# hideki1217/rusTfhe

Hardware: AMD Instinct MI355X
Metric: HomNAND gates/sec (whole node), N=1024 (higher is better)
Workload: dtype f64

## Files before the change

### rustfhe_amd/csrc/rtfhe_body_pair_rr.hpp

```cpp
    typedef PairRrLds S;
    constexpr int LOGN = 10, SLOTS = S::SLOTS;
    typedef Geo<LOGN> G;
    constexpr int N = G::N, P = G::P, R = G::R, NT = 128 * SLOTS;
    constexpr uint32_t MA = decomp_add(L, BGBIT, decltype(tvs)::ROUNDED), MX = decomp_xor(L, BGBIT, decltype(tvs)::ROUNDED);
    static_assert(L == 3, "three rows per side are held in registers");
    extern __shared__ __align__(16) unsigned char smem[];
    const int tid = threadIdx.x, lane = tid & 63;
    const int wave = __builtin_amdgcn_readfirstlane(tid >> 6);
    const int slot = wave % SLOTS;
    const int side = wave / SLOTS;
    const int per = a.count / (int)gridDim.x, extra = a.count % (int)gridDim.x, wg = (int)blockIdx.x;
    const int gc = per + (wg < extra ? 1 : 0);
    const int g_first = wg * per + (wg < extra ? wg : extra);
    if (gc < SLOTS || gc > S::GMAX) return;

    cplx* tw = reinterpret_cast<cplx*>(smem);
    for (int idx = tid; idx < G::TW_TOTAL; idx += NT) tw[idx] = a.tw[idx];
    const cplx* twf = tw;
    const cplx* twi = tw + G::TW_DIR;

    unsigned char* sbase = smem + S::TW + (size_t)slot * S::SLOT;
    double* xb0 = reinterpret_cast<double*>(sbase);
    double* xb1 = xb0 + 2 * G::XSLOTS;
    double* myx = side ? xb1 : xb0;
    cplx* hand0 = reinterpret_cast<cplx*>(xb0) + lane;
    cplx* hand1 = reinterpret_cast<cplx*>(xb1) + lane;
    uint32_t* flags = reinterpret_cast<uint32_t*>(sbase + 2 * S::XB);
    uint32_t* done = reinterpret_cast<uint32_t*>(smem + S::TW + SLOTS * S::SLOT);
    unsigned char* gates0 = smem + S::TW + SLOTS * S::SLOT + S::DONE;
    const size_t gate_bytes = S::gate_bytes(a.npad);
    if (lane == 0) flags[side] = 0u;
    if (tid < 2 * S::GMAX) done[tid] = 0u;
    const unsigned my_flag = (unsigned)__builtin_amdgcn_readfirstlane((int)(unsigned)(size_t)(__attribute__((address_space(3))) uint32_t*)(flags + side));
    const unsigned partner_flag = (unsigned)__builtin_amdgcn_readfirstlane((int)(unsigned)(size_t)(__attribute__((address_space(3))) uint32_t*)(flags + (1 - side)));
    const unsigned done_side = (unsigned)__builtin_amdgcn_readfirstlane((int)(unsigned)(size_t)(__attribute__((address_space(3))) uint32_t*)(done + side));

    const int n = a.n;
    for (int gl = 0; gl < gc; gl++) {
        constexpr int SH = 32 - LOGN - 1;
        const GateIo io = gate_io(a, g_first + gl);
        uint16_t* ab = reinterpret_cast<uint16_t*>(gates0 + gl * gate_bytes + (size_t)2 * N * 4);
        for (int i = tid; i <= n; i += NT) {
            const uint32_t t = gate_linear(io.op, io.p0[i], io.p1[i], i == n);
            if constexpr (decltype(tvs)::MANY) ab[i] = (uint16_t)mod_switch<SH>(t, i == n, tv_shift(tvs));
            else ab[i] = (uint16_t)((i == n) ? (t >> SH) : ((t + (1u << (SH - 1))) >> SH));
        }
    }
    __syncthreads();
    for (int gl = 0; gl < gc; gl++) {
        uint32_t* acc = reinterpret_cast<uint32_t*>(gates0 + gl * gate_bytes);
        const auto tv = tv_row(tvs, g_first + gl, N);
        const int bbar = (int)reinterpret_cast<const uint16_t*>(acc + 2 * N)[n];
        for (int c = tid; c < N; c += NT) {
            const int e = (c + bbar) & (2 * N - 1);
            acc[c] = tv_word<LOGN>(tv, e);
            if constexpr (decltype(tvs)::ENC) acc[N + c] = tv_word_a<LOGN>(tv, e);
            else acc[N + c] = 0u;
        }
    }
    __syncthreads();

    const size_t trgsw_cplx = (size_t)2 * L * 2 * R * 64;
    cplx bA[R], bB[R];
    typedef unsigned int v4u __attribute__((ext_vector_type(4)));
    const __amdgpu_buffer_rsrc_t bk_rsrc = __builtin_amdgcn_make_buffer_rsrc(const_cast<cplx*>(a.bk), 0, 0x7fffffff, 0x00020000);
    const int lane16 = lane * 16;
    auto fetch = [&](cplx (&dst)[R], int step, int rc) {
        const size_t row = (size_t)step * trgsw_cplx + (size_t)((side * L + rc % L) * 2 + rc / L) * R * 64;
        const int s_lo = __builtin_amdgcn_readfirstlane((int)(row * sizeof(cplx)));
        const int s_hi = s_lo + (R / 2) * 64 * (int)sizeof(cplx);
        __builtin_amdgcn_sched_barrier(0);
#pragma unroll
        for (int m = 0; m < R / 2; m++) {
            const v4u v = __builtin_amdgcn_raw_buffer_load_b128(bk_rsrc, lane16 + m * 1024, s_lo, 0);
            dst[m] = make_double2(__longlong_as_double(((unsigned long long)v.y << 32) | v.x), __longlong_as_double(((unsigned long long)v.w << 32) | v.z));
        }
#pragma unroll
        for (int m = 0; m < R / 2; m++) {
            const v4u v = __builtin_amdgcn_raw_buffer_load_b128(bk_rsrc, lane16 + m * 1024, s_hi, 0);
            dst[R / 2 + m] = make_double2(__longlong_as_double(((unsigned long long)v.y << 32) | v.x), __longlong_as_double(((unsigned long long)v.w << 32) | v.z));
        }
        __builtin_amdgcn_sched_barrier(0);
    };
    if (a.steps > 0) {
        fetch(bA, 0, side ? 0 : 1);
        fetch(bB, 0, side ? 1 : 0);
    }
    constexpr int LOWER_AT = 2, RAISE_AT = 10;
    auto prio_point = [&](int point) {
        if (point == LOWER_AT) asm volatile("s_cmp_lg_u32 %0, 0\n\ts_cbranch_scc1 1f\n\ts_setprio 0\n1:" ::"s"(side) : "scc");
        if (point == RAISE_AT) asm volatile("s_cmp_lg_u32 %0, 0\n\ts_cbranch_scc1 1f\n\ts_setprio 2\n1:" ::"s"(side) : "scc");
    };
    if (side) __builtin_amdgcn_s_setprio(1); else __builtin_amdgcn_s_setprio(2);
    unsigned seq = 0;
    int gl = slot, i = 0;
#pragma unroll 1
    while (i < a.steps) {
        int gl2 = gl + SLOTS, i2 = i;
        if (gl2 >= gc) { gl2 -= gc; i2++; }
        const int nxt = (i2 < a.steps) ? i2 : i;
        uint32_t* poly = reinterpret_cast<uint32_t*>(gates0 + gl * gate_bytes) + side * N;
        const int r = __builtin_amdgcn_readfirstlane((int)reinterpret_cast<const uint16_t*>(gates0 + gl * gate_bytes + (size_t)2 * N * 4)[i]);
        const unsigned done_flag = done_side + 8u * (unsigned)gl;
        flag_wait(done_flag, (unsigned)i);
        int ln = lane;
        asm volatile("" : "+v"(ln));
        uint32_t own[2 * R], u[2 * R];
#pragma unroll
        for (int mm = 0; mm < 2 * R; mm++) own[mm] = poly[ln + 64 * mm];
        rotated_gather(u, own, poly, ln, r, MA, MX);
        double xr[L][R], xi[L][R];
#pragma unroll
        for (int jj = 0; jj < L; jj++) {
#pragma unroll
            for (int m = 0; m < R; m++) {
                xr[jj][m] = (double)decomp_digit(u[m], BGBIT, jj);
                xi[jj][m] = (double)decomp_digit(u[R + m], BGBIT, jj);
            }
        }
        auto pp1 = [&]() { prio_point(1); };
        fft_forward_multi_a<LOGN, L, true, decltype(pp1), true>(xr, xi, twf, myx, myx + G::XSLOTS, ln, pp1);
        prio_point(2);
        fft_forward_multi_b<LOGN, L, BOOT_TRIV>(xr, xi, twf);
        prio_point(5);

        double sre[R], sim[R];
        auto zero = [&]() {
#pragma unroll
            for (int m = 0; m < R; m++) { sre[m] = 0.0; sim[m] = 0.0; }
        };
        auto put = [&](cplx* h) {
#pragma unroll
            for (int m = 0; m < R; m++) h[m * 64] = make_double2(sre[m], sim[m]);
        };
        auto get = [&](const cplx* h) {
#pragma unroll
            for (int m = 0; m < R; m++) { const cplx v = h[m * 64]; sre[m] = v.x; sim[m] = v.y; }
        };

        if (side == 0) {
            mac_row_first<R>(sre, sim, bB, xr[0], xi[0]); fetch(bB, i, 2);
            mac_row<R>(sre, sim, bA, xr[1], xi[1]); fetch(bA, i, 3);
            mac_row<R>(sre, sim, bB, xr[2], xi[2]); fetch(bB, i, 4);
            put(hand0);
        }
        prio_point(6);
        seq++; flag_arrive(my_flag, seq); flag_wait(partner_flag, seq);
        prio_point(7);
        if (side == 0) zero(); else get(hand0);
        mac_row<R>(sre, sim, bA, xr[0], xi[0]); fetch(bA, i, side ? 2 : 5);
        mac_row<R>(sre, sim, bB, xr[1], xi[1]); fetch(bB, side ? i : nxt, side ? 3 : 0);
        mac_row<R>(sre, sim, bA, xr[2], xi[2]); fetch(bA, side ? i : nxt, side ? 4 : 1);
        put(side ? hand0 : hand1);
        prio_point(8);
        seq++; flag_arrive(my_flag, seq); flag_wait(partner_flag, seq);
        prio_point(9);
        if (side == 1) {
            get(hand1);
            mac_row<R>(sre, sim, bB, xr[0], xi[0]); fetch(bB, i, 5);
            mac_row<R>(sre, sim, bA, xr[1], xi[1]); fetch(bA, nxt, 0);
            mac_row<R>(sre, sim, bB, xr[2], xi[2]); fetch(bB, nxt, 1);
        } else {
            get(hand0);
        }

        fft_inverse<LOGN, 1, BOOT_TRIV>(sre, sim, twi, twi, myx, lane);
#pragma unroll
        for (int m = 0; m < R; m++) {
            const int c = lane + 64 * m;
            poly[c] = own[m] + trunc_to_torus(sre[m]);
            poly[c + P] = own[R + m] + trunc_to_torus(sim[m]);
        }
        wave_lds_sync();
        flag_arrive(done_flag, (unsigned)i + 1u);
        prio_point(10);
        gl = gl2; i = i2;
    }
    __builtin_amdgcn_s_setprio(0);
    __syncthreads();

#define RR_PAIR_SYNC() do { seq++; flag_arrive(my_flag, seq); flag_wait(partner_flag, seq); } while (0)
#pragma unroll 1
    for (int ge_l = slot; ge_l < gc; ge_l += SLOTS) {
        const int g = g_first + ge_l;
        const GateIo io = gate_io(a, g, tvs);
        const bool live = io.ok;
        uint32_t* accbuf = reinterpret_cast<uint32_t*>(gates0 + ge_l * gate_bytes);
        uint32_t* poly = accbuf + side * N;
        if (a.mode == MODE_BLIND_ROTATE) {
            if (live) {
                uint32_t* o = a.out + (size_t)g * 2 * N + side * N;
                for (int c = lane; c < N; c += 64) o[c] = poly[c];
            }
            continue;
        }
        if (side == 1) {
            uint32_t av[2 * R];
#pragma unroll
            for (int mm = 0; mm < 2 * R; mm++) av[mm] = poly[lane + 64 * mm];
            wave_lds_sync();
#pragma unroll
            for (int mm = 0; mm < 2 * R; mm++) {
                const int c = lane + 64 * mm;
                poly[(N - c) & (N - 1)] = (c == 0) ? av[mm] : (0u - av[mm]);
            }
        }
        RR_PAIR_SYNC();
        if (a.mode == MODE_EXTRACT) {
            if constexpr (decltype(tvs)::MANY) {
                if (live) many_extract<N>(a.ext, a.ext_first + g, tv_shift(tvs), accbuf, side * (N / 2) + lane, (side + 1) * (N / 2), 64, side ? -1 : lane);
                continue;
            }
            if (live) {
                const int ge = a.ext_first + g;
                for (int c = side * (N / 2) + lane; c < (side + 1) * (N / 2); c += 64) *ext_slot(a.ext, ge, c, N) = accbuf[N + c];
                if (side == 0 && lane == 0) *ext_slot(a.ext, ge, N, N) = accbuf[0];
                for (int c = side * 64 + lane; c <= n; c += 128) io.out[c] = 0u;
            }
            continue;
        }
        uint4 sum[KSQ];
        ks_accumulate<LOGN, KS_T, KS_BB, KSQ>(accbuf + N, side * (N / 2), (side + 1) * (N / 2), a.ksk, a.ksw, sum, lane);
        uint4* part = reinterpret_cast<uint4*>(xb1) + lane;
        if (side == 1) {
#pragma unroll
            for (int q = 0; q < KSQ; q++) part[q * 64] = sum[q];
        }
        RR_PAIR_SYNC();
        if (side == 0 && live) {
            const uint32_t bprime = accbuf[0];
            uint32_t* out = io.out;
#pragma unroll
            for (int q = 0; q < KSQ; q++) {
                const uint4 o = part[q * 64];
                const int col = 4 * (lane + 64 * q);
                const uint32_t s[4] = {sum[q].x + o.x, sum[q].y + o.y, sum[q].z + o.z, sum[q].w + o.w};
#pragma unroll
                for (int e = 0; e < 4; e++)
                    if (col + e <= n) out[col + e] = ((col + e == n) ? bprime : 0u) - s[e];
            }
        }
        RR_PAIR_SYNC();
    }
#undef RR_PAIR_SYNC
```

### rustfhe_amd/csrc/rtfhe_device.hpp

```cpp
#pragma once

#include <hip/hip_runtime.h>
#include <stdint.h>

namespace rtfhe {

typedef double2 cplx;

constexpr bool BOOT_TRIV = true;

__host__ __device__ constexpr int ilog2(int v) { return v <= 1 ? 0 : 1 + ilog2(v >> 1); }

template <int LOGN>
struct Geo {
    static constexpr int N = 1 << LOGN;
    static constexpr int P = N / 2;
    static constexpr int LOGP = LOGN - 1;
    static constexpr int R = P / 64;
    static constexpr int LR = ilog2(R);
    static constexpr int LOW = LOGP - 2 * LR;
    static constexpr int NLOW = 1 << LOW;
    static_assert(LOW >= 2 && LOW <= LR, "supported: N = 1024, 2048");
    static constexpr int TW_TWIST = 0;
    static constexpr int TW_P1 = TW_TWIST + R * 64;
    static constexpr int TW_P2 = TW_P1 + (R - 1) * 64;
    static constexpr int TW_P3 = TW_P2 + (R - 1) * NLOW;
    static constexpr int TW_DIR = TW_P3 + (NLOW - 4);
    static constexpr int TW_TOTAL = 2 * TW_DIR;
    static constexpr int XSLOTS = P + 64;
    __host__ __device__ static constexpr int f1(int pos) { return pos + NLOW * (pos >> 6); }
    __host__ __device__ static constexpr int f2(int pos) { return pos + (pos >> LR); }
    __host__ __device__ static constexpr int pos1(int lane, int m) { return lane + 64 * m; }
    __host__ __device__ static constexpr int pos2(int lane, int m) {
        return ((lane >> LOW) << 6) | (m << LOW) | (lane & (NLOW - 1));
    }
    __host__ __device__ static constexpr int pos3(int lane, int m) { return (lane << LR) | m; }
};

__device__ __forceinline__ void wave_lds_sync() {
    __builtin_amdgcn_fence(__ATOMIC_RELEASE, "wavefront");
    __builtin_amdgcn_wave_barrier();
    __builtin_amdgcn_fence(__ATOMIC_ACQUIRE, "wavefront");
}

__device__ __forceinline__ void lds_st(double* p, double v) {
    __hip_atomic_store(p, v, __ATOMIC_RELAXED, __HIP_MEMORY_SCOPE_WAVEFRONT);
}
__device__ __forceinline__ double lds_ld(const double* p) {
    return __hip_atomic_load(p, __ATOMIC_RELAXED, __HIP_MEMORY_SCOPE_WAVEFRONT);
}
__device__ __forceinline__ void lds_st128(cplx* p, double re, double im) { *p = make_double2(re, im); }
__device__ __forceinline__ cplx lds_ld128(const cplx* p) { return *p; }


template <int CNT>
struct Tw {
    cplx w[CNT > 0 ? CNT : 1];
    __device__ __forceinline__ void load(const cplx* __restrict__ tw, int stride) {
#pragma unroll
        for (int e = 0; e < CNT; e++) w[e] = tw[e * stride];
    }
};

template <int R, int MB, bool TRIV0 = false>
__device__ __forceinline__ void fwd_stage_tw(double (&re)[R], double (&im)[R], const cplx* w) {
    constexpr int h = 1 << MB;
#pragma unroll
    for (int m = 0; m < R; m++) {
        if (m & h) continue;
        const int m1 = m | h, q = m & (h - 1);
        const double sr = re[m] + re[m1], si = im[m] + im[m1];
        const double dr = re[m] - re[m1], di = im[m] - im[m1];
        re[m] = sr; im[m] = si;
        if (TRIV0 && q == 0) { re[m1] = dr; im[m1] = di; continue; }
        double a = dr * w[q].x, b = di * w[q].y;
        re[m1] = a - b;
        a = dr * w[q].y; b = di * w[q].x;
        im[m1] = a + b;
    }
}

template <int R, int MB, bool CONJ = false, bool TRIV0 = false>
__device__ __forceinline__ void inv_stage_tw(double (&re)[R], double (&im)[R], const cplx* w) {
    constexpr int h = 1 << MB;
#pragma unroll
    for (int m = 0; m < R; m++) {
        if (m & h) continue;
        const int m1 = m | h, q = m & (h - 1);
        if (TRIV0 && q == 0) {
            const double ar = re[m], ai = im[m], tr = re[m1], ti = im[m1];
            re[m] = ar + tr; im[m] = ai + ti;
            re[m1] = ar - tr; im[m1] = ai - ti;
            continue;
        }
        const double t0 = re[m1] * w[q].x, t1 = re[m1] * w[q].y, t2 = im[m1] * w[q].x, t3 = im[m1] * w[q].y;
        const double tr = CONJ ? t0 + t3 : t0 - t3, ti = CONJ ? t2 - t1 : t1 + t2;
        const double ar = re[m], ai = im[m];
        re[m] = ar + tr; im[m] = ai + ti;
        re[m1] = ar - tr; im[m1] = ai - ti;
    }
}

template <int R>
__device__ __forceinline__ void stage_size2(double (&re)[R], double (&im)[R]) {
#pragma unroll
    for (int m = 0; m < R; m += 2) {
        const double r0 = re[m], r1 = re[m + 1], j0 = im[m], j1 = im[m + 1];
        re[m] = r0 + r1; re[m + 1] = r0 + (-r1);
        im[m] = j0 + j1; im[m + 1] = j0 + (-j1);
    }
}

template <int R>
__device__ __forceinline__ void fwd_stage_size4(double (&re)[R], double (&im)[R]) {
#pragma unroll
    for (int m = 0; m < R; m += 4) {
        const double r0 = re[m], r1 = re[m + 1], r2 = re[m + 2], r3 = re[m + 3];
        const double j0 = im[m], j1 = im[m + 1], j2 = im[m + 2], j3 = im[m + 3];
        re[m] = r0 + r2; re[m + 1] = r1 + r3; re[m + 2] = r0 + (-r2); re[m + 3] = (-j1) + j3;
        im[m] = j0 + j2; im[m + 1] = j1 + j3; im[m + 2] = j0 + (-j2); im[m + 3] = r1 + (-r3);
    }
}

template <int R>
__device__ __forceinline__ void inv_stage_size4(double (&re)[R], double (&im)[R]) {
#pragma unroll
    for (int m = 0; m < R; m += 4) {
        const double r0 = re[m], r1 = re[m + 1], r2 = re[m + 2], r3 = re[m + 3];
        const double j0 = im[m], j1 = im[m + 1], j2 = im[m + 2], j3 = im[m + 3];
        re[m] = r0 + r2; re[m + 1] = r1 + j3;    re[m + 2] = r0 + (-r2); re[m + 3] = r1 + (-j3);
        im[m] = j0 + j2; im[m + 1] = j1 + (-r3); im[m + 2] = j0 + (-j2); im[m + 3] = j1 + r3;
    }
}

template <int R>
__device__ __forceinline__ void twist_mul(double (&re)[R], double (&im)[R], const cplx* w) {
#pragma unroll
    for (int m = 0; m < R; m++) {
        const double rc = re[m] * w[m].x, ic = im[m] * w[m].x, rs = re[m] * w[m].y, is = im[m] * w[m].y;
        re[m] = rc - is;
        im[m] = ic + rs;
    }
}

template <int R, int MBTOP>
struct P12 {
    __device__ __forceinline__ static void fwd(double (&re)[R], double (&im)[R], const cplx* w) {
        if constexpr (MBTOP >= 0) {
            constexpr int h = 1 << MBTOP;
            fwd_stage_tw<R, MBTOP>(re, im, w + (R - 2 * h));
            P12<R, MBTOP - 1>::fwd(re, im, w);
        }
    }
    template <bool CONJ = false>
    __device__ __forceinline__ static void inv(double (&re)[R], double (&im)[R], const cplx* w) {
        if constexpr (MBTOP >= 0) {
            constexpr int h = 1 << MBTOP;
            P12<R, MBTOP - 1>::template inv<CONJ>(re, im, w);
            inv_stage_tw<R, MBTOP, CONJ>(re, im, w + (R - 2 * h));
        }
    }
};

template <int R, int NLOW, int MBTOP, bool TRIV = false>
struct P3 {
    __device__ __forceinline__ static void fwd(double (&re)[R], double (&im)[R], const cplx* w) {
        if constexpr (MBTOP >= 2) {
            constexpr int h = 1 << MBTOP;
            fwd_stage_tw<R, MBTOP, TRIV>(re, im, w + (NLOW - 2 * h));
            P3<R, NLOW, MBTOP - 1, TRIV>::fwd(re, im, w);
        } else {
            fwd_stage_size4<R>(re, im);
            stage_size2<R>(re, im);
        }
    }
    template <bool CONJ = false>
    __device__ __forceinline__ static void inv(double (&re)[R], double (&im)[R], const cplx* w) {
        if constexpr (MBTOP >= 2) {
            constexpr int h = 1 << MBTOP;
            P3<R, NLOW, MBTOP - 1, TRIV>::template inv<CONJ>(re, im, w);
            inv_stage_tw<R, MBTOP, CONJ, TRIV>(re, im, w + (NLOW - 2 * h));
        } else {
            stage_size2<R>(re, im);
            inv_stage_size4<R>(re, im);
        }
    }
};

template <int LOGN, int FROM, int TO, int DUAL = 0>
__device__ __forceinline__ void exchange(double (&re)[Geo<LOGN>::R], double (&im)[Geo<LOGN>::R],
                                         double* __restrict__ xbuf, int lane, double* __restrict__ ximbuf = nullptr) {
    typedef Geo<LOGN> G;
    constexpr int R = G::R;
    auto slot = [&](int layout, int m) {
        const int pos = layout == 1 ? G::pos1(lane, m) : layout == 2 ? G::pos2(lane, m) : G::pos3(lane, m);
        return (FROM + TO == 3) ? G::f1(pos) : G::f2(pos);
    };
    if constexpr (DUAL && G::LR == G::LOW) {
        double* xim = ximbuf ? ximbuf : xbuf + G::XSLOTS;
        constexpr bool X12 = (FROM + TO == 3);
        auto base = [&](int layout) {
            return layout == 1 ? lane : layout == 2 ? (G::NLOW + 64) * (lane >> G::LOW) + (lane & (G::NLOW - 1)) : (R + 1) * lane;
        };
        auto stride = [](int layout) constexpr { return layout == 1 ? 64 + G::NLOW : layout == 2 ? (X12 ? G::NLOW : G::NLOW + 1) : 1; };
        static_assert(G::f1(G::pos1(5, 3)) == 5 + (64 + G::NLOW) * 3 && G::f2(G::pos3(5, 3)) == (R + 1) * 5 + 3, "affine slot maps");
        const int bw = base(FROM), br = base(TO);
        constexpr int sw = stride(FROM), sr = stride(TO);
        if constexpr (DUAL == 2) {
            cplx* xc = reinterpret_cast<cplx*>(xbuf);
#pragma unroll
            for (int m = 0; m < R; m++) lds_st128(&xc[bw + sw * m], re[m], im[m]);
            wave_lds_sync();
#pragma unroll
            for (int m = 0; m < R / 2; m++) {
                const cplx a = lds_ld128(&xc[br + sr * m]), b = lds_ld128(&xc[br + sr * (m + R / 2)]);
                re[m] = a.x; im[m] = a.y; re[m + R / 2] = b.x; im[m + R / 2] = b.y;
            }
            wave_lds_sync();
            return;
        }
#pragma unroll
        for (int m = 0; m < R; m++) lds_st(&xbuf[bw + sw * m], re[m]);
#pragma unroll
        for (int m = 0; m < R; m++) lds_st(&xim[bw + sw * m], im[m]);
        wave_lds_sync();
#pragma unroll
        for (int m = 0; m < R / 2; m++) {
            re[m] = lds_ld(&xbuf[br + sr * m]); re[m + R / 2] = lds_ld(&xbuf[br + sr * (m + R / 2)]);
            im[m] = lds_ld(&xim[br + sr * m]);  im[m + R / 2] = lds_ld(&xim[br + sr * (m + R / 2)]);
        }
        wave_lds_sync();
    } else if constexpr (DUAL) {
        double* xim = ximbuf ? ximbuf : xbuf + G::XSLOTS;
#pragma unroll
        for (int m = 0; m < R; m++) lds_st(&xbuf[slot(FROM, m)], re[m]);
#pragma unroll
        for (int m = 0; m < R; m++) lds_st(&xim[slot(FROM, m)], im[m]);
        wave_lds_sync();
#pragma unroll
        for (int m = 0; m < R / 2; m++) {
            re[m] = lds_ld(&xbuf[slot(TO, m)]); re[m + R / 2] = lds_ld(&xbuf[slot(TO, m + R / 2)]);
            im[m] = lds_ld(&xim[slot(TO, m)]);  im[m + R / 2] = lds_ld(&xim[slot(TO, m + R / 2)]);
        }
        wave_lds_sync();
    } else {
#pragma unroll
        for (int m = 0; m < R; m++) lds_st(&xbuf[slot(FROM, m)], re[m]);
        wave_lds_sync();
#pragma unroll
        for (int m = 0; m < R; m++) re[m] = lds_ld(&xbuf[slot(TO, m)]);
        wave_lds_sync();
#pragma unroll
        for (int m = 0; m < R; m++) lds_st(&xbuf[slot(FROM, m)], im[m]);
        wave_lds_sync();
#pragma unroll
        for (int m = 0; m < R; m++) im[m] = lds_ld(&xbuf[slot(TO, m)]);
        wave_lds_sync();
    }
}

template <int LOGN, int DUAL = 0>
__device__ __forceinline__ void fft_forward_a(double (&re)[Geo<LOGN>::R], double (&im)[Geo<LOGN>::R],
                                              const cplx* __restrict__ tw, double* __restrict__ xbuf, int lane,
                                              double* __restrict__ xim = nullptr) {
    typedef Geo<LOGN> G;
    constexpr int R = G::R;
    Tw<R> wt; Tw<R - 1> w1, w2;
    wt.load(tw + G::TW_TWIST + lane, 64);
    w1.load(tw + G::TW_P1 + lane, 64);
    twist_mul<R>(re, im, wt.w);
    P12<R, G::LR - 1>::fwd(re, im, w1.w);
    w2.load(tw + G::TW_P2 + (lane & (G::NLOW - 1)), G::NLOW);
    exchange<LOGN, 1, 2, DUAL>(re, im, xbuf, lane, xim);
    P12<R, G::LR - 1>::fwd(re, im, w2.w);
}
template <int LOGN, int DUAL = 0, bool TRIV = false>
__device__ __forceinline__ void fft_forward_b(double (&re)[Geo<LOGN>::R], double (&im)[Geo<LOGN>::R],
                                              const cplx* __restrict__ tw, double* __restrict__ xbuf, int lane,
                                              double* __restrict__ xim = nullptr) {
    typedef Geo<LOGN> G;
    Tw<G::NLOW - 4> w3;
    w3.load(tw + G::TW_P3, 1);
    exchange<LOGN, 2, 3, DUAL>(re, im, xbuf, lane, xim);
    P3<G::R, G::NLOW, G::LOW - 1, TRIV>::fwd(re, im, w3.w);
}
template <int LOGN, int DUAL = 0, bool TRIV = false>
__device__ __forceinline__ void fft_forward(double (&re)[Geo<LOGN>::R], double (&im)[Geo<LOGN>::R],
                                            const cplx* __restrict__ tw, double* __restrict__ xbuf, int lane,
                                            double* __restrict__ xim = nullptr) {
    fft_forward_a<LOGN, DUAL>(re, im, tw, xbuf, lane, xim);
    fft_forward_b<LOGN, DUAL, TRIV>(re, im, tw, xbuf, lane, xim);
}

template <int LOGN, int FROM, int TO, bool B128 = false>
struct XAffine {
    typedef Geo<LOGN> G;
    static_assert(G::LR == G::LOW, "N = 1024 geometry");
    static constexpr int R = G::R;
    static constexpr bool X12 = (FROM + TO == 3);
    __device__ __forceinline__ static int base(int layout, int lane) {
        return layout == 1 ? lane : layout == 2 ? (G::NLOW + 64) * (lane >> G::LOW) + (lane & (G::NLOW - 1)) : (R + 1) * lane;
    }
    __host__ __device__ static constexpr int stride(int layout) { return layout == 1 ? 64 + G::NLOW : layout == 2 ? (X12 ? G::NLOW : G::NLOW + 1) : 1; }
    __device__ __forceinline__ static void write(const double (&re)[R], const double (&im)[R], double* __restrict__ xbuf, double* __restrict__ xim, int lane) {
        const int bw = base(FROM, lane);
        constexpr int sw = stride(FROM);
        if constexpr (B128) {
            cplx* xc = reinterpret_cast<cplx*>(xbuf);
#pragma unroll
            for (int m = 0; m < R; m++) lds_st128(&xc[bw + sw * m], re[m], im[m]);
            return;
        }
#pragma unroll
        for (int m = 0; m < R; m++) lds_st(&xbuf[bw + sw * m], re[m]);
#pragma unroll
        for (int m = 0; m < R; m++) lds_st(&xim[bw + sw * m], im[m]);
    }
    template <int HALF>
    __device__ __forceinline__ static void read_half(double (&re)[R], double (&im)[R], const double* __restrict__ xbuf, const double* __restrict__ xim, int lane) {
        const int br = base(TO, lane);
        constexpr int sr = stride(TO);
        if constexpr (B128) {
            const cplx* xc = reinterpret_cast<const cplx*>(xbuf);
#pragma unroll
            for (int m = HALF * (R / 4); m < (HALF + 1) * (R / 4); m++) {
                const cplx a = lds_ld128(&xc[br + sr * m]), b = lds_ld128(&xc[br + sr * (m + R / 2)]);
                re[m] = a.x; im[m] = a.y; re[m + R / 2] = b.x; im[m + R / 2] = b.y;
            }
            return;
        }
#pragma unroll
        for (int m = HALF * (R / 4); m < (HALF + 1) * (R / 4); m++) {
            re[m] = lds_ld(&xbuf[br + sr * m]); re[m + R / 2] = lds_ld(&xbuf[br + sr * (m + R / 2)]);
            im[m] = lds_ld(&xim[br + sr * m]);  im[m + R / 2] = lds_ld(&xim[br + sr * (m + R / 2)]);
        }
    }
};

struct NoHook { __device__ __forceinline__ void operator()() const {} };
template <int LOGN, int NR, bool TWIST = true, typename HOOK = NoHook, bool INTERLEAVE = false, bool B128 = false>
__device__ __forceinline__ void fft_forward_multi_a(double (&re)[NR][Geo<LOGN>::R], double (&im)[NR][Geo<LOGN>::R],
                                                    const cplx* __restrict__ tw, double* __restrict__ xbuf, double* __restrict__ xim, int lane,
                                                    HOOK after_pass1 = HOOK()) {
    typedef Geo<LOGN> G;
    constexpr int R = G::R;
#pragma unroll
    for (int half = 0; half < (TWIST ? 2 : 0); half++) {
        cplx wt[R / 2];
#pragma unroll
        for (int m = 0; m < R / 2; m++) wt[m] = tw[G::TW_TWIST + lane + 64 * (half * (R / 2) + m)];
#pragma unroll
        for (int j = 0; j < NR; j++)
#pragma unroll
            for (int m = 0; m < R / 2; m++) {
                const int k = half * (R / 2) + m;
                const double rc = re[j][k] * wt[m].x, ic = im[j][k] * wt[m].x, rs = re[j][k] * wt[m].y, is = im[j][k] * wt[m].y;
                re[j][k] = rc - is;
                im[j][k] = ic + rs;
            }
    }
  if constexpr (INTERLEAVE) {
    static_assert(G::LR == 3, "three stages per pass");
    typedef XAffine<LOGN, 1, 2, B128> X1;
    typedef XAffine<LOGN, 2, 3, B128> X2;
    auto pass = [&](int j, const cplx* w, auto&& between0, auto&& between1) {
        fwd_stage_tw<R, 2>(re[j], im[j], w + (R - 8));
        __builtin_amdgcn_sched_barrier(0); between0(); __builtin_amdgcn_sched_barrier(0);
        fwd_stage_tw<R, 1>(re[j], im[j], w + (R - 4));
        __builtin_amdgcn_sched_barrier(0); between1(); __builtin_amdgcn_sched_barrier(0);
        fwd_stage_tw<R, 0>(re[j], im[j], w + (R - 2));
        __builtin_amdgcn_sched_barrier(0);
    };
    auto nothing = [] {};
    Tw<R - 1> w1;
    w1.load(tw + G::TW_P1 + lane, 64);
#pragma unroll
    for (int j = 0; j < NR; j++) {
        if (j == 0) pass(0, w1.w, nothing, nothing);
        else pass(j, w1.w, [&] { X1::template read_half<0>(re[j - 1], im[j - 1], xbuf, xim, lane); }, [&] { X1::template read_half<1>(re[j - 1], im[j - 1], xbuf, xim, lane); wave_lds_sync(); });
        X1::write(re[j], im[j], xbuf, xim, lane);
        wave_lds_sync();
    }
    after_pass1();
    Tw<R - 1> w2;
    w2.load(tw + G::TW_P2 + (lane & (G::NLOW - 1)), G::NLOW);
#pragma unroll
    for (int j = 0; j < NR; j++) {
        if (j == 0) pass(0, w2.w, [&] { X1::template read_half<0>(re[NR - 1], im[NR - 1], xbuf, xim, lane); }, [&] { X1::template read_half<1>(re[NR - 1], im[NR - 1], xbuf, xim, lane); wave_lds_sync(); });
        else pass(j, w2.w, [&] { X2::template read_half<0>(re[j - 1], im[j - 1], xbuf, xim, lane); }, [&] { X2::template read_half<1>(re[j - 1], im[j - 1], xbuf, xim, lane); wave_lds_sync(); });
        X2::write(re[j], im[j], xbuf, xim, lane);
        wave_lds_sync();
    }
    X2::template read_half<0>(re[NR - 1], im[NR - 1], xbuf, xim, lane);
    X2::template read_half<1>(re[NR - 1], im[NR - 1], xbuf, xim, lane);
    wave_lds_sync();
  } else {
    {
        Tw<R - 1> w1;
        w1.load(tw + G::TW_P1 + lane, 64);
#pragma unroll
        for (int j = 0; j < NR; j++) {
            P12<R, G::LR - 1>::fwd(re[j], im[j], w1.w);
            exchange<LOGN, 1, 2, B128 ? 2 : 1>(re[j], im[j], xbuf, lane, xim);
        }
    }
    after_pass1();
    Tw<R - 1> w2;
    w2.load(tw + G::TW_P2 + (lane & (G::NLOW - 1)), G::NLOW);
#pragma unroll
    for (int j = 0; j < NR; j++) {
        P12<R, G::LR - 1>::fwd(re[j], im[j], w2.w);
        exchange<LOGN, 2, 3, B128 ? 2 : 1>(re[j], im[j], xbuf, lane, xim);
    }
  }
}
template <int LOGN, int NR, bool TRIV = false>
__device__ __forceinline__ void fft_forward_multi_b(double (&re)[NR][Geo<LOGN>::R], double (&im)[NR][Geo<LOGN>::R],
                                                    const cplx* __restrict__ tw) {
    typedef Geo<LOGN> G;
    Tw<G::NLOW - 4> w3;
    w3.load(tw + G::TW_P3, 1);
#pragma unroll
    for (int j = 0; j < NR; j++) P3<G::R, G::NLOW, G::LOW - 1, TRIV>::fwd(re[j], im[j], w3.w);
}

template <int LOGN, int DUAL = 0, bool TRIV = false>
__device__ __forceinline__ void fft_inverse(double (&re)[Geo<LOGN>::R], double (&im)[Geo<LOGN>::R],
                                            const cplx* __restrict__ tw_small, const cplx* __restrict__ tw_big,
                                            double* __restrict__ xbuf, int lane, double* __restrict__ xim = nullptr) {
    typedef Geo<LOGN> G;
    constexpr int R = G::R;
    Tw<G::NLOW - 4> w3; Tw<R - 1> w2, w1; Tw<R> wt;
    w3.load(tw_small + G::TW_P3, 1);
    P3<R, G::NLOW, G::LOW - 1, TRIV>::template inv<false>(re, im, w3.w);
    w2.load(tw_small + G::TW_P2 + (lane & (G::NLOW - 1)), G::NLOW);
    exchange<LOGN, 3, 2, DUAL>(re, im, xbuf, lane, xim);
    P12<R, G::LR - 1>::inv(re, im, w2.w);
    w1.load(tw_big + G::TW_P1 + lane, 64);
    exchange<LOGN, 2, 1, DUAL>(re, im, xbuf, lane, xim);
    wt.load(tw_big + G::TW_TWIST + lane, 64);
    P12<R, G::LR - 1>::inv(re, im, w1.w);
    twist_mul<R>(re, im, wt.w);
}

template <int LOGN>
struct TwStage {
    typedef Geo<LOGN> G;
    static constexpr bool SPLIT = (LOGN >= 11);
    static constexpr int LDS_CPLX = SPLIT ? G::TW_DIR + (G::TW_DIR - G::TW_P2) : G::TW_TOTAL;
    __device__ __forceinline__ static void stage(cplx* __restrict__ lds, const cplx* __restrict__ global, int tid, int nthreads) {
        if constexpr (SPLIT) {
            for (int idx = tid; idx < G::TW_DIR; idx += nthreads) lds[idx] = global[idx];
            for (int idx = tid + G::TW_P2; idx < G::TW_DIR; idx += nthreads) lds[G::TW_DIR + idx - G::TW_P2] = global[G::TW_DIR + idx];
        } else {
            for (int idx = tid; idx < G::TW_TOTAL; idx += nthreads) lds[idx] = global[idx];
        }
    }
    __device__ __forceinline__ static const cplx* fwd(const cplx* lds) { return lds; }
    __device__ __forceinline__ static const cplx* inv_small(const cplx* lds) { return SPLIT ? lds + G::TW_DIR - G::TW_P2 : lds + G::TW_DIR; }
    __device__ __forceinline__ static const cplx* inv_big(const cplx* lds, const cplx* global) { return SPLIT ? global + G::TW_DIR : lds + G::TW_DIR; }
};

__device__ __forceinline__ uint32_t trunc_to_torus(double x) {
    const double t = __builtin_trunc(x);
    const double y = t + 6755399441055744.0;
    return (uint32_t)__double_as_longlong(y);
}

__device__ __forceinline__ uint32_t trunc_to_torus_wide(double x) {
    const double t = __builtin_trunc(x);
    if (!(__builtin_fabs(t) < 9223372036854775808.0)) return 0u;
    const double hi = __builtin_floor(t * 2.3283064365386963e-10);
    const double lo = __builtin_fma(hi, -4294967296.0, t);
    return (uint32_t)lo;
}

__host__ __device__ constexpr uint32_t decomp_mask(int l, int bits) {
    uint32_t u = 0;
    if (32 - l * bits != 0) {
        u += 1u << (32 - l * bits - 1);
        for (int i = l; i >= 1; i--) u += 1u << (32 - i * bits - 1);
    } else {
        for (int i = l - 1; i >= 1; i--) u += 1u << (32 - i * bits - 1);
    }
    return u;
}

__host__ __device__ constexpr uint32_t decomp_xor(int l, int bits, bool rounded) {
    if (!rounded) return decomp_mask(l, bits);
    uint32_t u = 0;
    for (int j = 1; j <= l; j++) u += 1u << (32 - bits * j + bits - 1);
    return u;
}
__host__ __device__ constexpr uint32_t decomp_add(int l, int bits, bool rounded) {
    if (!rounded) return decomp_mask(l, bits);
    return decomp_xor(l, bits, true) + (32 - l * bits != 0 ? 1u << (32 - l * bits - 1) : 0u);
}
static_assert(decomp_xor(3, 6, true) == 0x82080000u && decomp_add(3, 6, true) == 0x82082000u, "rounded decomposition, l = 3, bgbit = 6");
static_assert(decomp_xor(3, 6, false) == 0x02084000u && decomp_add(3, 6, false) == 0x02084000u, "reference decomposition, l = 3, bgbit = 6");

__device__ __forceinline__ int32_t decomp_digit(uint32_t u, int bits, int j) {
    return __builtin_amdgcn_sbfe((int32_t)u, (uint32_t)(32 - bits * (j + 1)), (uint32_t)bits);
}


__device__ __forceinline__ void flag_arrive(unsigned flag, unsigned k) {
    unsigned t0, t1;
    asm volatile("v_mov_b32 %0, %2\n\tv_mov_b32 %1, %3\n\tds_write_b32 %0, %1" : "=&v"(t0), "=&v"(t1) : "s"(flag), "s"(k) : "memory");
}
__device__ __forceinline__ void flag_wait(unsigned flag, unsigned k) {
    unsigned v, t;
    asm volatile(
        "v_mov_b32 %0, %2\n"
        "1:\n\t"
        "ds_read_b32 %0, %0\n\t"
        "s_waitcnt lgkmcnt(0)\n\t"
        "v_readfirstlane_b32 %1, %0\n\t"
        "s_sub_i32 %1, %1, %3\n\t"
        "s_cmp_lt_i32 %1, 0\n\t"
        "s_cbranch_scc0 2f\n\t"
        "s_sleep 1\n\t"
        "v_mov_b32 %0, %2\n\t"
        "s_branch 1b\n"
        "2:"
        : "=&v"(v), "=&s"(t)
        : "s"(flag), "s"(k)
        : "memory", "scc");
}
template <int LOGN>
__device__ __forceinline__ uint32_t rotated_coef(const uint32_t* __restrict__ p, int c, int r) {
    constexpr int N = 1 << LOGN;
    const int e = (c - r) & (2 * N - 1);
    const uint32_t v = p[e & (N - 1)];
    return (e >> LOGN) ? (0u - v) : v;
}

template <int Q>
__device__ __forceinline__ void rotated_gather_case(uint32_t (&u)[16], const uint32_t (&own)[16], const uint32_t* __restrict__ p1,
                                                    const uint32_t* __restrict__ p2, uint32_t s, uint32_t sx, uint32_t ma, uint32_t mx) {
    const uint32_t k0 = ma - s, k1 = ma - ~s;
#pragma unroll
    for (int mm = 0; mm < 16; mm++) {
        const int blk = (mm - Q) & 15;
        if (blk == 0) {
            u[mm] = ((p2[0] ^ sx) + ((ma - sx) - own[mm])) ^ mx;
        } else if (mm < Q) {
            u[mm] = ((p1[64 * blk] ^ ~s) + (k1 - own[mm])) ^ mx;
        } else {
            u[mm] = ((p1[64 * blk] ^ s) + (k0 - own[mm])) ^ mx;
        }
    }
}
__device__ __forceinline__ void rotated_gather(uint32_t (&u)[16], const uint32_t (&own)[16], const uint32_t* __restrict__ p, int ln, int r,
                                               uint32_t ma, uint32_t mx) {
    const int q = r >> 6, d = ln - (r & 63);
    const bool neg = d < 0;
    const int base = 4 * (d & 63) - (neg ? 256 : 0);
    const uint32_t* p1 = reinterpret_cast<const uint32_t*>(reinterpret_cast<const unsigned char*>(p) + base);
    const uint32_t* p2 = reinterpret_cast<const uint32_t*>(reinterpret_cast<const unsigned char*>(p) + base + (neg ? 4096 : 0));
    const uint32_t s = 0u - (uint32_t)(q >> 4), sx = s ^ (neg ? ~0u : 0u);
    switch (q & 15) {
#define RTFHE_GATHER_CASE(Q) case Q: rotated_gather_case<Q>(u, own, p1, p2, s, sx, ma, mx); break;
        RTFHE_GATHER_CASE(0) RTFHE_GATHER_CASE(1) RTFHE_GATHER_CASE(2) RTFHE_GATHER_CASE(3)
        RTFHE_GATHER_CASE(4) RTFHE_GATHER_CASE(5) RTFHE_GATHER_CASE(6) RTFHE_GATHER_CASE(7)
        RTFHE_GATHER_CASE(8) RTFHE_GATHER_CASE(9) RTFHE_GATHER_CASE(10) RTFHE_GATHER_CASE(11)
        RTFHE_GATHER_CASE(12) RTFHE_GATHER_CASE(13) RTFHE_GATHER_CASE(14) RTFHE_GATHER_CASE(15)
#undef RTFHE_GATHER_CASE
    }
}

}
```

Before: 160,800.

## Interleave accumulator halves in LDS as 64-bit pairs for paired loads/stores

Changes the LDS layout of each accumulator side so that coefficient c and c+N/2 sit adjacent as one 64-bit word, via a pair_word index map. The blind-rotate loop now loads and stores real/imag halves with a single 64-bit LDS access, and uses a new rotated_gather_pairs that fetches pairs and swaps halves on wraparound. The epilogue unpacks the pair layout back to linear order before output and extraction. This halves the LDS instruction count in the hot loop but adds select logic in the gather and an extra unpack pass in the epilogue.

```diff
diff --git a/rustfhe_amd/csrc/rtfhe_body_pair_rr.hpp b/rustfhe_amd/csrc/rtfhe_body_pair_rr.hpp
--- a/rustfhe_amd/csrc/rtfhe_body_pair_rr.hpp
+++ b/rustfhe_amd/csrc/rtfhe_body_pair_rr.hpp
@@ -1,7 +1,7 @@
     typedef PairRrLds S;
     constexpr int LOGN = 10, SLOTS = S::SLOTS;
     typedef Geo<LOGN> G;
-    constexpr int N = G::N, P = G::P, R = G::R, NT = 128 * SLOTS;
+    constexpr int N = G::N, R = G::R, NT = 128 * SLOTS;
     constexpr uint32_t MA = decomp_add(L, BGBIT, decltype(tvs)::ROUNDED), MX = decomp_xor(L, BGBIT, decltype(tvs)::ROUNDED);
     static_assert(L == 3, "three rows per side are held in registers");
     extern __shared__ __align__(16) unsigned char smem[];
@@ -53,9 +53,9 @@
         const int bbar = (int)reinterpret_cast<const uint16_t*>(acc + 2 * N)[n];
         for (int c = tid; c < N; c += NT) {
             const int e = (c + bbar) & (2 * N - 1);
-            acc[c] = tv_word<LOGN>(tv, e);
-            if constexpr (decltype(tvs)::ENC) acc[N + c] = tv_word_a<LOGN>(tv, e);
-            else acc[N + c] = 0u;
+            acc[pair_word(c)] = tv_word<LOGN>(tv, e);
+            if constexpr (decltype(tvs)::ENC) acc[N + pair_word(c)] = tv_word_a<LOGN>(tv, e);
+            else acc[N + pair_word(c)] = 0u;
         }
     }
     __syncthreads();
@@ -107,8 +107,11 @@
         asm volatile("" : "+v"(ln));
         uint32_t own[2 * R], u[2 * R];
 #pragma unroll
-        for (int mm = 0; mm < 2 * R; mm++) own[mm] = poly[ln + 64 * mm];
-        rotated_gather(u, own, poly, ln, r, MA, MX);
+        for (int m = 0; m < R; m++) {
+            const unsigned long long v = pair_load(poly, ln + 64 * m);
+            own[m] = (uint32_t)v; own[R + m] = (uint32_t)(v >> 32);
+        }
+        rotated_gather_pairs(u, own, poly, ln, r, MA, MX);
         double xr[L][R], xi[L][R];
 #pragma unroll
         for (int jj = 0; jj < L; jj++) {
@@ -166,11 +169,7 @@
 
         fft_inverse<LOGN, 1, BOOT_TRIV>(sre, sim, twi, twi, myx, lane);
 #pragma unroll
-        for (int m = 0; m < R; m++) {
-            const int c = lane + 64 * m;
-            poly[c] = own[m] + trunc_to_torus(sre[m]);
-            poly[c + P] = own[R + m] + trunc_to_torus(sim[m]);
-        }
+        for (int m = 0; m < R; m++) pair_store(poly, lane + 64 * m, own[m] + trunc_to_torus(sre[m]), own[R + m] + trunc_to_torus(sim[m]));
         wave_lds_sync();
         flag_arrive(done_flag, (unsigned)i + 1u);
         prio_point(10);
@@ -187,18 +186,25 @@
         const bool live = io.ok;
         uint32_t* accbuf = reinterpret_cast<uint32_t*>(gates0 + ge_l * gate_bytes);
         uint32_t* poly = accbuf + side * N;
+        uint32_t av[2 * R];
+#pragma unroll
+        for (int m = 0; m < R; m++) {
+            const unsigned long long v = pair_load(poly, lane + 64 * m);
+            av[m] = (uint32_t)v; av[R + m] = (uint32_t)(v >> 32);
+        }
+        wave_lds_sync();
         if (a.mode == MODE_BLIND_ROTATE) {
             if (live) {
                 uint32_t* o = a.out + (size_t)g * 2 * N + side * N;
-                for (int c = lane; c < N; c += 64) o[c] = poly[c];
+#pragma unroll
+                for (int mm = 0; mm < 2 * R; mm++) o[lane + 64 * mm] = av[mm];
             }
             continue;
         }
-        if (side == 1) {
-            uint32_t av[2 * R];
-#pragma unroll
-            for (int mm = 0; mm < 2 * R; mm++) av[mm] = poly[lane + 64 * mm];
-            wave_lds_sync();
+        if (side == 0) {
+#pragma unroll
+            for (int mm = 0; mm < 2 * R; mm++) poly[lane + 64 * mm] = av[mm];
+        } else {
 #pragma unroll
             for (int mm = 0; mm < 2 * R; mm++) {
                 const int c = lane + 64 * mm;
diff --git a/rustfhe_amd/csrc/rtfhe_device.hpp b/rustfhe_amd/csrc/rtfhe_device.hpp
--- a/rustfhe_amd/csrc/rtfhe_device.hpp
+++ b/rustfhe_amd/csrc/rtfhe_device.hpp
@@ -569,4 +569,50 @@
     }
 }
 
-}
+__host__ __device__ constexpr int pair_word(int k) { return 2 * (k & 511) + (k >> 9); }
+__device__ __forceinline__ void pair_store(uint32_t* p, int slot, uint32_t lo, uint32_t hi) {
+    __hip_atomic_store(reinterpret_cast<unsigned long long*>(p) + slot, ((unsigned long long)hi << 32) | lo, __ATOMIC_RELAXED, __HIP_MEMORY_SCOPE_WAVEFRONT);
+}
+__device__ __forceinline__ unsigned long long pair_load(const uint32_t* p, int slot) {
+    return __hip_atomic_load(reinterpret_cast<const unsigned long long*>(p) + slot, __ATOMIC_RELAXED, __HIP_MEMORY_SCOPE_WAVEFRONT);
+}
+template <int Q>
+__device__ __forceinline__ void rotated_gather_pairs_case(uint32_t (&u)[16], const uint32_t (&own)[16], const uint32_t* __restrict__ p1,
+                                                          const uint32_t* __restrict__ p2, bool neg, uint32_t s, uint32_t sx, uint32_t ma, uint32_t mx) {
+    const uint32_t k0 = ma - s, k1 = ma - ~s;
+#pragma unroll
+    for (int mm = 0; mm < 8; mm++) {
+        const int blk = (mm - Q) & 15, B = blk & 7, h = blk >> 3;
+        const unsigned long long v = B ? pair_load(p1, 64 * B) : pair_load(p2, 0);
+        uint32_t w0 = (uint32_t)v, w1 = (uint32_t)(v >> 32);
+        if (B == 0) {
+            const uint32_t a0 = neg ? w1 : w0, a1 = neg ? w0 : w1;
+            w0 = a0; w1 = a1;
+        }
+        const uint32_t lo = h ? w1 : w0, hi = h ? w0 : w1;
+        if (blk == 0) u[mm] = ((lo ^ sx) + ((ma - sx) - own[mm])) ^ mx;
+        else if (mm < Q) u[mm] = ((lo ^ ~s) + (k1 - own[mm])) ^ mx;
+        else u[mm] = ((lo ^ s) + (k0 - own[mm])) ^ mx;
+        if (blk == 8) u[mm + 8] = ((hi ^ sx) + ((ma - sx) - own[mm + 8])) ^ mx;
+        else if (mm + 8 < Q) u[mm + 8] = ((hi ^ ~s) + (k1 - own[mm + 8])) ^ mx;
+        else u[mm + 8] = ((hi ^ s) + (k0 - own[mm + 8])) ^ mx;
+    }
+}
+__device__ __forceinline__ void rotated_gather_pairs(uint32_t (&u)[16], const uint32_t (&own)[16], const uint32_t* __restrict__ p, int ln, int r,
+                                                     uint32_t ma, uint32_t mx) {
+    const int q = r >> 6, d = ln - (r & 63);
+    const bool neg = d < 0;
+    const uint32_t* p1 = reinterpret_cast<const uint32_t*>(reinterpret_cast<const unsigned char*>(p) + 8 * d);
+    const uint32_t* p2 = reinterpret_cast<const uint32_t*>(reinterpret_cast<const unsigned char*>(p) + 8 * d + (neg ? 4096 : 0));
+    const uint32_t s = 0u - (uint32_t)(q >> 4), sx = s ^ (neg ? ~0u : 0u);
+    switch (q & 15) {
+#define RTFHE_GATHER_CASE(Q) case Q: rotated_gather_pairs_case<Q>(u, own, p1, p2, neg, s, sx, ma, mx); break;
+        RTFHE_GATHER_CASE(0) RTFHE_GATHER_CASE(1) RTFHE_GATHER_CASE(2) RTFHE_GATHER_CASE(3)
+        RTFHE_GATHER_CASE(4) RTFHE_GATHER_CASE(5) RTFHE_GATHER_CASE(6) RTFHE_GATHER_CASE(7)
+        RTFHE_GATHER_CASE(8) RTFHE_GATHER_CASE(9) RTFHE_GATHER_CASE(10) RTFHE_GATHER_CASE(11)
+        RTFHE_GATHER_CASE(12) RTFHE_GATHER_CASE(13) RTFHE_GATHER_CASE(14) RTFHE_GATHER_CASE(15)
+#undef RTFHE_GATHER_CASE
+    }
+}
+
+}
```

Measured after the change: 160,700. Within noise of the previous version (-0.1%).
